# klasmodin/quflow

Measured on AMD Instinct MI355X. Metric: isospectral timesteps/sec at N=1024 (1 GPU) + ensemble steps/sec at 1/2/4/8 GPUs, higher is better.
Workload: dtype f64

## Files before the change

### include/quflow_hip.h

```cpp
#ifndef QUFLOW_HIP_H
#define QUFLOW_HIP_H

#ifdef __cplusplus
extern "C" {
#endif

#define QF_OK 0
#define QF_ERR_INVALID 1
#define QF_ERR_NO_DEVICE 2
#define QF_ERR_HIP 3
#define QF_ERR_STATE 4
#define QF_ERR_CALLBACK 5
#define QF_ERR_UNSUPPORTED 6
#define QF_ERR_NONFINITE 7

#define QF_VERSION 100

typedef struct qf_ctx qf_ctx;

int qf_version(void);
const char *qf_last_error(void);
int qf_device_count(void);

int qf_ctx_create(int N, int device, qf_ctx **out);
// ... 96 lines not shown
#define QF_KERNEL_UPDATE 4
#define QF_KERNEL_SLICE 5
#define QF_KERNEL_COUNT 6

int qf_profile_enable(qf_ctx *ctx, int mask);
int qf_profile_reset(qf_ctx *ctx);
int qf_profile_read(qf_ctx *ctx, int kernel_id, long long *launches, double *total_ms);
int qf_profile_stride(qf_ctx *ctx, int stride);
int qf_profile_seen(qf_ctx *ctx, int kernel_id, long long *seen);
int qf_device_info(int device, char *buf, int n);
int qf_plan_describe(qf_ctx *ctx, char *buf, int n);
int qf_timer_start(qf_ctx *ctx);
int qf_timer_stop(qf_ctx *ctx, double *elapsed_ms);

#define QF_BUF_W 0
#define QF_BUF_DW 1
#define QF_BUF_WHALF 2
#define QF_BUF_PHALF 3
#define QF_BUF_PW 4
int qf_download_buffer(qf_ctx *ctx, int which, void *host);
int qf_debug_guard_check(long long *allocations, long long *damaged, char *first, int n);
int qf_debug_modulus(qf_ctx *ctx, int n, const double *er_host, const double *ei_host, double *out_modulus_host,
                     double *out_sqrt_host);
int qf_zgemm(qf_ctx *ctx, const void *A_host, const void *B_host, void *C_host);
int qf_commutator(qf_ctx *ctx, const void *W_host, const void *P_host, void *C_host, int skewherm);
int qf_zgemm_i8(qf_ctx *ctx, const void *A_host, const void *B_host, void *C_host);
int qf_fixedpoint_products(qf_ctx *ctx, const void *Phalf_host, const void *Whalf_host, const void *W_host,
                           const void *dW_old_host, int variant, void *dW_new_host, void *Whalf_new_host,
                           double *rowsum_host);

int qf_c64_laplacian_table(qf_ctx *ctx, int bc, float *lap_host);
int qf_c64_solve_poisson(qf_ctx *ctx, const void *W_host, void *P_host, int skewh);
int qf_c64_solve_tridiagonal(qf_ctx *ctx, const float *lap_host, const void *W_host, void *P_host, int skewh);
int qf_c64_laplace(qf_ctx *ctx, const void *P_host, void *W_host);
int qf_c64_upload_W(qf_ctx *ctx, const void *W_host);
int qf_c64_download_W(qf_ctx *ctx, void *W_host);
int qf_c64_isomp(qf_ctx *ctx, double dt, int steps, double tol, int minit, int maxit, int compsum, int reinitialize,
                 qf_isomp_stats *stats_out);
int qf_c64_isomp_continue(qf_ctx *ctx, double dt, int steps, double tol, int minit, int maxit, int compsum, int reinitialize,
                          qf_isomp_stats *stats_out);
int qf_c64_diagnostics(qf_ctx *ctx, double *energy_euler, double *enstrophy);
int qf_cgemm(qf_ctx *ctx, const void *A_host, const void *B_host, void *C_host);
int qf_c64_fixedpoint_products(qf_ctx *ctx, const void *Phalf_host, const void *Whalf_host, const void *W_host,
                               const void *dW_old_host, void *dW_new_host, void *Whalf_new_host, double *rowsum_host);
int qf_c64_fixedpoint_products_tri(qf_ctx *ctx, const void *Phalf_host, const void *Whalf_host, const void *W_host,
                                   const void *dW_old_host, void *dW_new_host, void *Whalf_new_host, double *rowsum_host);
// ... 14 lines not shown
```

### quflow_amd/_lib.py

```python
import ctypes
import os

_HERE = os.path.dirname(os.path.abspath(__file__))
LIB_PATH = os.environ.get("QUFLOW_HIP_LIB") or os.path.join(_HERE, "libquflow_hip.so")

QF_OK = 0
QF_ERR_NONFINITE = 7
ERR_NAMES = {1: "QF_ERR_INVALID", 2: "QF_ERR_NO_DEVICE", 3: "QF_ERR_HIP", 4: "QF_ERR_STATE", 5: "QF_ERR_CALLBACK",
             6: "QF_ERR_UNSUPPORTED", 7: "QF_ERR_NONFINITE"}

KERNEL_IDS = {"poisson": 0, "gemm1": 1, "gemm2": 2, "norm": 3, "update": 4, "slice": 5}
ERK_METHODS = {"euler": 0, "heun": 1, "rk4": 2}
BUFFER_IDS = {"W": 0, "dW": 1, "Whalf": 2, "Phalf": 3, "PW": 4}


class QuflowHipError(RuntimeError):
    pass


HAMILTONIAN_CB = ctypes.CFUNCTYPE(ctypes.c_int, ctypes.c_void_p, ctypes.c_void_p, ctypes.c_void_p, ctypes.c_double)
FORCING_CB = ctypes.CFUNCTYPE(ctypes.c_int, ctypes.c_void_p, ctypes.c_void_p, ctypes.c_void_p, ctypes.c_void_p, ctypes.c_double)
STRANG_CB = ctypes.CFUNCTYPE(ctypes.c_int, ctypes.c_void_p, ctypes.c_double, ctypes.c_void_p)
CALLBACK_CB = ctypes.CFUNCTYPE(ctypes.c_int, ctypes.c_void_p, ctypes.c_void_p, ctypes.c_void_p)

# ... 76 lines not shown
                                            ctypes.POINTER(IsompHooks)]),
    "qf_basis_upload": (ctypes.c_int, [_vp, _vp, ctypes.c_longlong]),
    "qf_basis_compute": (ctypes.c_int, [_vp]),
    "qf_basis_download": (ctypes.c_int, [_vp, _vp, ctypes.c_longlong]),
    "qf_basis_stream": (ctypes.c_int, [_vp, ctypes.c_longlong]),
    "qf_basis_slab_plan": (ctypes.c_int, [ctypes.c_int, ctypes.c_int, ctypes.c_longlong, ctypes.POINTER(ctypes.c_int),
                                          ctypes.c_int]),
    "qf_shr2mat": (ctypes.c_int, [_vp, _vp, ctypes.c_longlong, _vp]),
    "qf_mat2shr": (ctypes.c_int, [_vp, _vp, _vp, ctypes.c_longlong]),
    "qf_shc2mat": (ctypes.c_int, [_vp, _vp, _vp]),
    "qf_mat2shc": (ctypes.c_int, [_vp, _vp, _vp]),
    "qf_shr2fun": (ctypes.c_int, [_vp, _vp, ctypes.c_longlong, ctypes.c_int, ctypes.c_int, _vp]),
    "qf_shc2fun": (ctypes.c_int, [_vp, _vp, ctypes.c_longlong, ctypes.c_int, ctypes.c_int, ctypes.c_int, _vp]),
    "qf_fun2shc": (ctypes.c_int, [_vp, _vp, ctypes.c_int, ctypes.c_int, _vp]),
    "qf_fun2shr": (ctypes.c_int, [_vp, _vp, ctypes.c_int, ctypes.c_int, _vp]),
    "qf_diagnostics": (ctypes.c_int, [_vp, _dp, _dp]),
    "qf_norm_inf_W": (ctypes.c_int, [_vp, _dp]),
    "qf_profile_enable": (ctypes.c_int, [_vp, ctypes.c_int]),
    "qf_profile_reset": (ctypes.c_int, [_vp]),
    "qf_profile_read": (ctypes.c_int, [_vp, ctypes.c_int, ctypes.POINTER(ctypes.c_longlong), _dp]),
    "qf_plan_describe": (ctypes.c_int, [_vp, ctypes.c_char_p, ctypes.c_int]),
    "qf_device_info": (ctypes.c_int, [ctypes.c_int, ctypes.c_char_p, ctypes.c_int]),
    "qf_debug_modulus": (ctypes.c_int, [_vp, ctypes.c_int, _dp, _dp, _dp, _dp]),
    "qf_profile_stride": (ctypes.c_int, [_vp, ctypes.c_int]),
    "qf_profile_seen": (ctypes.c_int, [_vp, ctypes.c_int, ctypes.POINTER(ctypes.c_longlong)]),
    "qf_timer_start": (ctypes.c_int, [_vp]),
    "qf_timer_stop": (ctypes.c_int, [_vp, _dp]),
    "qf_download_buffer": (ctypes.c_int, [_vp, ctypes.c_int, _vp]),
    "qf_debug_guard_check": (ctypes.c_int, [ctypes.POINTER(ctypes.c_longlong), ctypes.POINTER(ctypes.c_longlong), ctypes.c_char_p, ctypes.c_int]),
    "qf_zgemm": (ctypes.c_int, [_vp, _vp, _vp, _vp]),
    "qf_commutator": (ctypes.c_int, [_vp, _vp, _vp, _vp, ctypes.c_int]),
    "qf_zgemm_i8": (ctypes.c_int, [_vp, _vp, _vp, _vp]),
    "qf_fixedpoint_products": (ctypes.c_int, [_vp, _vp, _vp, _vp, _vp, ctypes.c_int, _vp, _vp, _vp]),
    "qf_c64_laplacian_table": (ctypes.c_int, [_vp, ctypes.c_int, _vp]),
    "qf_c64_solve_poisson": (ctypes.c_int, [_vp, _vp, _vp, ctypes.c_int]),
    "qf_c64_laplace": (ctypes.c_int, [_vp, _vp, _vp]),
    "qf_c64_solve_tridiagonal": (ctypes.c_int, [_vp, _vp, _vp, _vp, ctypes.c_int]),
    "qf_c64_upload_W": (ctypes.c_int, [_vp, _vp]),
    "qf_c64_download_W": (ctypes.c_int, [_vp, _vp]),
    "qf_c64_isomp": (ctypes.c_int, [_vp, ctypes.c_double, ctypes.c_int, ctypes.c_double, ctypes.c_int,
                                    ctypes.c_int, ctypes.c_int, ctypes.c_int, ctypes.POINTER(IsompStats)]),
    "qf_c64_isomp_continue": (ctypes.c_int, [_vp, ctypes.c_double, ctypes.c_int, ctypes.c_double, ctypes.c_int,
                                             ctypes.c_int, ctypes.c_int, ctypes.c_int, ctypes.POINTER(IsompStats)]),
    "qf_c64_diagnostics": (ctypes.c_int, [_vp, _dp, _dp]),
    "qf_cgemm": (ctypes.c_int, [_vp, _vp, _vp, _vp]),
    "qf_c64_fixedpoint_products": (ctypes.c_int, [_vp, _vp, _vp, _vp, _vp, _vp, _vp, _vp]),
# ... 45 lines not shown
```

### quflow_amd/csrc/api_context.hip

```cpp
#include <cmath>
#include <cstdarg>
#include <cstdio>
#include <cstdlib>
#include <cstring>
#include <limits>
#include <chrono>

#include "qf_api.h"

static thread_local char g_err[512] = "";

void qf_set_error(const char *fmt, ...)
{
    va_list ap;
    va_start(ap, fmt);
    vsnprintf(g_err, sizeof(g_err), fmt, ap);
    va_end(ap);
}

extern "C" {

int qf_version(void) { return QF_VERSION; }

int qf_device_info(int device, char *buf, int n)
// ... 133 lines not shown
    ctx->rowpart_tiles = qf_gemm_tiles_n(N);
    {
        const int slots32 = (N + 31) / 32;
        QF_CREATE_HIP(hipMalloc((void **)&ctx->rowpart, (size_t)(ctx->rowpart_tiles > slots32 ? ctx->rowpart_tiles : slots32) * N * sizeof(double)));
    }
    QF_CREATE_HIP(hipMalloc((void **)&ctx->rowsum, (size_t)N * sizeof(double)));
    QF_CREATE_HIP(hipMalloc((void **)&ctx->scalars, 4096 * sizeof(double)));
    QF_CREATE_HIP(hipHostMalloc((void **)&ctx->host_scalars, 64 * sizeof(double), hipHostMallocDefault));
    QF_CREATE_HIP(hipMalloc((void **)&ctx->state, sizeof(qf_dev_state)));
    QF_CREATE_HIP(hipMemsetAsync(ctx->state, 0, sizeof(qf_dev_state), ctx->stream));
    QF_CREATE_HIP(hipMalloc((void **)&ctx->ticket, 704 * sizeof(unsigned)));
    QF_CREATE_HIP(hipMemsetAsync(ctx->ticket, 0, 704 * sizeof(unsigned), ctx->stream));
    QF_CREATE_HIP(hipHostMalloc((void **)&ctx->host_rec, sizeof(qf_host_record), hipHostMallocCoherent));
    memset(ctx->host_rec, 0, sizeof(qf_host_record));
    {
        hipDeviceProp_t prop;
        QF_CREATE_HIP(hipGetDeviceProperties(&prop, device));
        ctx->num_cus = prop.multiProcessorCount;
        if (N % 64 == 0 && ctx->num_cus > 0) {
            ctx->sk_slots = ctx->num_cus;
            QF_CREATE_HIP(hipMalloc((void **)&ctx->sk_partial, (size_t)ctx->sk_slots * 64 * 64 * sizeof(cplx)));
            QF_CREATE_HIP(hipMalloc((void **)&ctx->sk_flags, (size_t)(ctx->sk_slots + 16) * sizeof(unsigned)));
            QF_CREATE_HIP(hipMemsetAsync(ctx->sk_flags, 0, (size_t)(ctx->sk_slots + 16) * sizeof(unsigned), ctx->stream));
        }
    }
    QF_CREATE_HIP(hipEventCreate(&ctx->timer_start));
    QF_CREATE_HIP(hipEventCreate(&ctx->timer_stop));
#undef QF_CREATE_HIP
    if ((rc = alloc_factors(ctx, &ctx->poisson)) != QF_OK) return fail(rc);
    if ((rc = qf_launch_lap_table(ctx, 1, ctx->lap)) != QF_OK) return fail(rc);
    if ((rc = qf_launch_build_factors(ctx, ctx->lap, ctx->poisson)) != QF_OK) return fail(rc);
    if (hipStreamSynchronize(ctx->stream) != hipSuccess) {
        qf_set_error("qf_ctx_create: table construction failed");
        return fail(QF_ERR_HIP);
    }
    *out = ctx;
    return QF_OK;
}

int qf_ctx_destroy(qf_ctx *ctx)
{
    if (!ctx) return QF_OK;
    (void)hipSetDevice(ctx->device);
    if (ctx->stream) (void)hipStreamSynchronize(ctx->stream);
    void *ptrs[] = {ctx->W, ctx->dW[0], ctx->dW[1], ctx->Whalf, ctx->Phalf, ctx->PW, ctx->kahan_c, ctx->stage,
                    ctx->lap, ctx->lap_user, ctx->poisson.tab, ctx->rowpart, ctx->rowsum,
                    ctx->t32_partial, ctx->t32_arrive, ctx->W2, ctx->Whalf2, ctx->ns_inv, ctx->ns_tmp, ctx->multi_rowpart, ctx->scalars, ctx->sk_partial, ctx->sk_flags, ctx->basis, ctx->sh_stage, ctx->sh_omega, ctx->slab};
    for (void *p : ptrs)
        if (p) (void)hipFree(p);
    void *sht[] = {ctx->sht.omega, ctx->sht.tab, ctx->sht.col, ctx->sht.At, ctx->sht.tw, ctx->sht.f, ctx->sht.H, ctx->sht.Q};
    for (void *p : sht)
        if (p) (void)hipFree(p);
    for (cplx *p : ctx->multi)
        if (p) (void)hipFree(p);
    for (int q = 0; q < 4; ++q) {
        if (ctx->oz_planes[q]) (void)hipFree(ctx->oz_planes[q]);
        if (ctx->oz_scale[q]) (void)hipFree(ctx->oz_scale[q]);
        if (q == 0 && ctx->oz_tbuf) (void)hipFree(ctx->oz_tbuf);
        if (q == 0 && ctx->oz_tflags) (void)hipFree(ctx->oz_tflags);
        if (q == 0 && ctx->oz_diag) (void)hipFree(ctx->oz_diag);
    }
    for (auto &kv : ctx->user_factors) {
        if (kv.second.f.tab) (void)hipFree(kv.second.f.tab);
    }
    for (int q = 0; q < 3; ++q)
        if (ctx->hook_host[q]) (void)hipHostFree(ctx->hook_host[q]);
    qf_c64_free(ctx->c64);
    ctx->c64 = nullptr;
    if (ctx->host_scalars) (void)hipHostFree(ctx->host_scalars);
    if (ctx->host_rec) (void)hipHostFree(ctx->host_rec);
// ... 160 lines not shown
int qf_download_buffer(qf_ctx *ctx, int which, void *host)
{
    QF_TRY(check_ctx(ctx));
    const cplx *src = nullptr;
    switch (which) {
        case QF_BUF_W: src = ctx->W; break;
        case QF_BUF_DW: src = ctx->dW[ctx->dw_cur]; break;
        case QF_BUF_WHALF: src = ctx->Whalf; break;
        case QF_BUF_PHALF: src = ctx->Phalf; break;
        case QF_BUF_PW: src = ctx->PW; break;
        default:
            qf_set_error("qf_download_buffer: unknown buffer %d", which);
            return QF_ERR_INVALID;
    }
    if (!host) {
        qf_set_error("qf_download_buffer: null host pointer");
        return QF_ERR_INVALID;
    }
    QF_HIP(hipMemcpyAsync(host, src, (size_t)ctx->N * ctx->N * sizeof(cplx), hipMemcpyDeviceToHost, ctx->stream));
    QF_HIP(hipStreamSynchronize(ctx->stream));
    return QF_OK;
}

int qf_debug_modulus(qf_ctx *ctx, int n, const double *er_host, const double *ei_host, double *out_modulus_host,
                     double *out_sqrt_host)
{
    QF_TRY(check_ctx(ctx));
    if (n < 1 || (size_t)n > (size_t)ctx->N * ctx->N || !er_host || !ei_host || !out_modulus_host || !out_sqrt_host) {
        qf_set_error("qf_debug_modulus: bad arguments (n=%d)", n);
        return QF_ERR_INVALID;
    }
    double *d = reinterpret_cast<double *>(ctx->stage), *o = reinterpret_cast<double *>(ctx->PW);
    QF_HIP(hipMemcpyAsync(d, er_host, (size_t)n * sizeof(double), hipMemcpyHostToDevice, ctx->stream));
    QF_HIP(hipMemcpyAsync(d + n, ei_host, (size_t)n * sizeof(double), hipMemcpyHostToDevice, ctx->stream));
    QF_TRY(qf_launch_debug_modulus(ctx, n, d, d + n, o, o + n));
    QF_HIP(hipMemcpyAsync(out_modulus_host, o, (size_t)n * sizeof(double), hipMemcpyDeviceToHost, ctx->stream));
    QF_HIP(hipMemcpyAsync(out_sqrt_host, o + n, (size_t)n * sizeof(double), hipMemcpyDeviceToHost, ctx->stream));
    QF_HIP(hipStreamSynchronize(ctx->stream));
    return QF_OK;
}


}
```

### quflow_amd/csrc/qf_internal.h

```cpp
#pragma once

#include <hip/hip_runtime.h>

#include <atomic>
#include <cstdarg>
#include <cstdio>
#include <map>
#include <mutex>
#include <string>
#include <vector>

#include "../../include/quflow_hip.h"

typedef double2 cplx;

hipError_t qf_guard_malloc(void **p, size_t bytes);
hipError_t qf_guard_free(void *p);
#define hipMalloc(p, n) qf_guard_malloc((void **)(p), (n))
#define hipFree(p) qf_guard_free((void *)(p))

void qf_set_error(const char *fmt, ...);
struct qf_ctx;
inline void qf_plan_note(qf_ctx *ctx, unsigned long long key, const char *fmt, ...) __attribute__((format(printf, 3, 4)));

// ... 255 lines not shown
    int rowpart_tiles = 0;
    double *rowsum = nullptr;
    double *scalars = nullptr;
    double *host_scalars = nullptr;
    qf_dev_state *state = nullptr;
    qf_host_record *host_rec = nullptr;
    bool diag_at_exit = false, diag_valid = false;
    unsigned *ticket = nullptr;
    int pred_iters = 3;
    bool gemm_tri_allowed = true;
    bool gemm_tri = false;
    int gemm_tri_min_n = 960;
    bool gemm_tri32 = false;
    int tri32_split = 2, tri32_split_diag = 1;
    cplx *t32_partial = nullptr;
    unsigned *t32_arrive = nullptr;
    bool defer_allowed = true;
    bool defer = false;
    int num_cus = 0;
    cplx *sk_partial = nullptr;
    unsigned *sk_flags = nullptr;
    int sk_slots = 0;
    unsigned sk_epoch = 0;
    int sk_epi_units = 0;
    int sk_epi_units_fused = 2;
    int sk_min_units = 8;
    int debug_drop = 0;
    bool needs_reset = false;

    qf_c64 *c64 = nullptr;

    int profile_mask = 0;
    std::vector<qf_event_pair> events_busy;
    std::vector<qf_event_pair> events_free;
    int profile_stride = 1;
    struct plan_slot {
        unsigned long long key = 0;
        char text[384] = {0};
    } plan[QF_KERNEL_COUNT];
    int plan_role = -1;
    long long prof_seen[QF_KERNEL_COUNT] = {0};
    long long prof_launches[QF_KERNEL_COUNT] = {0};
    double prof_ms[QF_KERNEL_COUNT] = {0};
    hipEvent_t timer_start = nullptr, timer_stop = nullptr;
};

// ... 37 lines not shown
    cplx *Whalf = nullptr;
    double *rowpart = nullptr;
    int fused = 0;
    cplx *Wpair[2] = {nullptr, nullptr};
    cplx *Whalf_step = nullptr;
    unsigned *ticket = nullptr;
    int n_tiles = 0;
    qf_dev_state *state_rw = nullptr;
    qf_host_record *rec = nullptr;
    int debug_drop = 0;
};
struct qf_streamk {
    cplx *partial = nullptr;
    unsigned *flags = nullptr;
    unsigned epoch = 0;
    int *fault = nullptr;
    unsigned *ticket = nullptr;
    int n_tiles = 0;
    qf_dev_state *state_rw = nullptr;
    qf_host_record *rec = nullptr;
    unsigned spin_limit = 1u << 22;
    int debug_drop = 0;
    int slots = 0;
};
struct qf_tri32 {
    cplx *partial = nullptr;
    unsigned *arrive = nullptr;
    int split = 1;
    int split_diag = 1;
    unsigned *ticket = nullptr;
    int n_tiles = 0;
    qf_dev_state *state_rw = nullptr;
    qf_host_record *rec = nullptr;
    int debug_drop = 0;
    int deferred = 0;
};
int qf_gemm_tiles_n(int N);
int qf_launch_zgemm_tri32(qf_ctx *ctx, const cplx *A, const cplx *B, const qf_epilogue *ep, qf_guard guard = qf_guard());
int qf_launch_zgemm_tri(qf_ctx *ctx, const cplx *A, const cplx *B, const qf_epilogue *ep, qf_guard guard = qf_guard());
int qf_launch_zgemm(qf_ctx *ctx, const cplx *A, const cplx *B, cplx *C, const qf_epilogue *ep,
                    qf_guard guard = qf_guard());

int qf_launch_basis(qf_ctx *ctx, double *basis_dev);
__host__ __device__ inline long long qf_slab_prefix(int N, int Nmax, int m)
{
    const long long a = m, n = N, k = Nmax;
    return a * n * k - (n + k) * (a * (a - 1) / 2) + (a - 1) * a * (2 * a - 1) / 6;
// ... 64 lines not shown
```

### quflow_amd/csrc/qf_step_end.h

```cpp
#pragma once

#include "qf_internal.h"

template <int ROWS = 4>
__device__ inline void qf_fused_step_end(int N, int slots, const double *rowpart, unsigned *ticket, qf_dev_state *state,
                                  qf_host_record *rec, int g_iter, int tid, double *scratch)
{
    double *part = scratch;
    int *nanflag = reinterpret_cast<int *>(scratch + 4);
    const bool check = (g_iter + 1 >= state->minit);
    double mx = 0.0;
    int nan = 0;
    if (check) {
        typedef unsigned v2u __attribute__((ext_vector_type(2)));
        const __amdgpu_buffer_rsrc_t rs_rp = __builtin_amdgcn_make_buffer_rsrc(
            const_cast<double *>(rowpart), 0, (int)((size_t)slots * N * sizeof(double)), 0x00020000);
        const unsigned slot_bytes = (unsigned)((size_t)N * sizeof(double));
        for (int ib = tid; ib < N; ib += ROWS * 256) {
            double sum[ROWS];
#pragma unroll
            for (int r = 0; r < ROWS; ++r) sum[r] = 0.0;
            for (int t0 = 0; t0 < slots; t0 += 16) {
                v2u v[ROWS][16];
#pragma unroll
                for (int r = 0; r < ROWS; ++r) {
// ... 7 lines not shown
#pragma unroll
                for (int r = 0; r < ROWS; ++r)
#pragma unroll
                    for (int t = 0; t < 16; ++t)
                        if (t0 + t < slots) sum[r] += *reinterpret_cast<const double *>(&v[r][t]);
            }
#pragma unroll
            for (int r = 0; r < ROWS; ++r)
                if (ib + 256 * r < N) {
                    if (sum[r] != sum[r]) nan = 1; else mx = fmax(mx, sum[r]);
                }
        }
#pragma unroll
        for (int off = 32; off > 0; off >>= 1) {
            mx = fmax(mx, __shfl_xor(mx, off, 64));
            nan |= __shfl_xor(nan, off, 64);
        }
        if ((tid & 63) == 0) {
            part[tid >> 6] = mx;
            nanflag[tid >> 6] = nan;
        }
    }
    __syncthreads();
    if (tid == 0) {
        __hip_atomic_store(ticket, 0u, __ATOMIC_RELAXED, __HIP_MEMORY_SCOPE_AGENT);
        const int iters = g_iter + 1;
        state->total_iterations += 1;
        state->dw_parity ^= 1;
        bool done = false, aborted = false;
        if (check) {
            double r = fmax(fmax(part[0], part[1]), fmax(part[2], part[3]));
            if (nanflag[0] | nanflag[1] | nanflag[2] | nanflag[3]) r = __builtin_nan("");
            const double resnorm_old = state->resnorm;
            state->resnorm = r;
            if (!QF_FINITE(r)) aborted = true;
            if (r <= state->tol || r >= resnorm_old) done = true;
        }
        if (aborted) {
            rec->nonfinite = 1;
            rec->last_step_iters = iters;
            rec->resnorm = state->resnorm;
            state->step_index = QF_STEP_ABORTED;
            state->iters_this_step = 0;
            state->wh_sel = 0;
        } else if (done || iters >= state->maxit) {
            if (!done) state->number_of_maxit += 1;
            rec->last_step_iters = iters;
            rec->resnorm = state->resnorm;
            state->step_index += 1;
            state->iters_this_step = 0;
            state->resnorm = __builtin_inf();
            state->w_parity ^= 1;
            state->wh_sel = 1;
        } else {
            state->iters_this_step = iters;
            state->wh_sel = 0;
        }
        rec->total_iterations = state->total_iterations;
        rec->number_of_maxit = state->number_of_maxit;
        rec->step_index = state->step_index;
        rec->w_parity = state->w_parity;
        rec->wh_sel = state->wh_sel;
        rec->dw_parity = state->dw_parity;
        const unsigned long long prog = ((unsigned long long)(unsigned)state->step_index << 32) |
                                        (unsigned long long)(unsigned)state->iters_this_step;
        __hip_atomic_store(&rec->progress, prog, __ATOMIC_RELEASE, __HIP_MEMORY_SCOPE_SYSTEM);
    }
}



struct qf_new_state {
    int step_index, iters_this_step, wh_sel, w_parity, dw_parity;
    int closed, last_step_iters, hit_maxit;
    int nonfinite;
    double resnorm;
    double last_resnorm;
};

__device__ inline qf_new_state qf_decide_compute(int N, int slots, const double *__restrict__ rowpart,
                                                 const qf_dev_state *st, double *scratch)
{
    const int tid = threadIdx.x, nth = blockDim.x, nw = nth >> 6;
    double *part = scratch;
    int *nanflag = reinterpret_cast<int *>(scratch + 20);
    const int iters = st->pending_iter + 1;
    const int minit = st->minit, maxit = st->maxit;
    const double tol = st->tol, resnorm_old = st->resnorm;
    const int step_index = st->step_index, w_parity = st->w_parity, dw_parity = st->dw_parity;
    const bool check = iters >= minit;
    double r = 0.0;
    {
        double mx = 0.0;
// ... 102 lines not shown
```

### quflow_amd/csrc/zgemm.hip

```cpp
#include "qf_internal.h"
#include "qf_step_end.h"

#include <cstring>

typedef double v4d __attribute__((ext_vector_type(4)));

#ifdef QF_STAMP
__device__ unsigned long long *qf_stamp_buf = nullptr;
#define QF_STAMP_SLOTS 80
#ifdef QF_STAMP_LIGHT
#define QF_STAMP_AT(slot_)
#define QF_STAMP_PH(kt_, ph_)
__device__ unsigned long long *qf_phase_buf = nullptr;
#else
#define QF_STAMP_AT(slot_)                                                              \
    if (qf_stamp_buf && lane == 0 && (slot_) < QF_STAMP_SLOTS)                          \
        qf_stamp_buf[((size_t)blockIdx.x * (T / 64) + wave) * QF_STAMP_SLOTS + (slot_)] = __builtin_amdgcn_s_memtime();
__device__ unsigned long long *qf_phase_buf = nullptr;
#define QF_STAMP_PH(kt_, ph_)                                                           \
    if (qf_phase_buf && tid == 0 && (kt_) >= 20 && (kt_) < 28)                          \
        qf_phase_buf[((size_t)blockIdx.x * 8 + ((kt_) - 20)) * 5 + (ph_)] = __builtin_amdgcn_s_memtime();
#endif
__device__ unsigned long long *qf_tri_buf = nullptr;
#define QF_TRI_STAMP(seg_, k_)                                                          \
    if (qf_tri_buf && tid == 0 && (seg_) < 4)                                           \
        qf_tri_buf[((size_t)blockIdx.x * 4 + (seg_)) * 8 + (k_)] = __builtin_amdgcn_s_memtime();
#define QF_TRI_NOTE(seg_, k_, v_)                                                       \
    if (qf_tri_buf && tid == 0 && (seg_) < 4) qf_tri_buf[((size_t)blockIdx.x * 4 + (seg_)) * 8 + (k_)] = (unsigned long long)(v_);
#else
#define QF_STAMP_AT(slot_)
#define QF_STAMP_PH(kt_, ph_)
#define QF_TRI_STAMP(seg_, k_)
#define QF_TRI_NOTE(seg_, k_, v_)
#endif
#ifndef QF_ABL_NOSTORE
#define QF_ABL_NOSTORE 0
#endif
#ifndef QF_ABL_NOSUMS
#define QF_ABL_NOSUMS 0
#endif
#ifndef QF_ABL_NOADD
#define QF_ABL_NOADD 0
#endif
#define QF_SUM3M(c_) (QF_ABL_NOADD ? (c_).x : (c_).x + (c_).y)
#ifndef QF_ABL_NOGLOAD
#define QF_ABL_NOGLOAD 0
#endif
#ifndef QF_ABL_NOBARRIER
#define QF_ABL_NOBARRIER 0
#endif
#ifndef QF_SK_AUX_ST
// ... 803 lines not shown
                            }
                        }
                    }
                    asm volatile("s_barrier" ::: "memory");
                    const unsigned soff = (unsigned)((size_t)slot2 * (BM * BN) * sizeof(cplx));
                    cplx v[MT * NT * 4];
#pragma unroll
                    for (int q = 0; q < MT * NT * 4; ++q) {
                        const v4u raw = __builtin_amdgcn_raw_buffer_load_b128(rsrcP, p_voff + (unsigned)(q * T * sizeof(cplx)), soff, QF_SK_AUX_LD);
                        v[q] = *reinterpret_cast<const cplx *>(&raw);
                    }
#pragma unroll
                    for (int mi = 0; mi < MT; ++mi)
#pragma unroll
                        for (int ni = 0; ni < NT; ++ni)
#pragma unroll
                            for (int reg = 0; reg < 4; ++reg) {
                                tre[mi][ni][reg] += v[(mi * NT + ni) * 4 + reg].x;
                                tim[mi][ni][reg] += v[(mi * NT + ni) * 4 + reg].y;
                            }
                }
            }
            QF_TRI_STAMP(seg, 2)
            cplx *Th = reinterpret_cast<cplx *>(smem_raw);
            cplx *Ts = reinterpret_cast<cplx *>(smem_raw + TT_BYTES);
            double *rs = reinterpret_cast<double *>(smem_raw + 2 * TT_BYTES);
            double *cs = rs + WN * BM;
            unsigned *open_flag = reinterpret_cast<unsigned *>(cs + WM * BN);
            const bool offdiag = (tm != tn);
            asm volatile("s_waitcnt lgkmcnt(0)\n\ts_barrier" ::: "memory");

            double csum[NT] = {0.0, 0.0};
            if (tid == 0) *open_flag = 0u;
#pragma unroll
            for (int mi = 0; mi < MT; ++mi) {
#pragma unroll
                for (int reg = 0; reg < 4; ++reg) {
                    const int li = wm * WTM + mi * 16 + q4 + 4 * reg;
                    double rsum = 0.0;
#pragma unroll
                    for (int ni = 0; ni < NT; ++ni) {
                        const int lj = wn * WTN + ni * 16 + r16;
                        const size_t e = (size_t)(i0 + li) * N + (j0 + lj);
                        const double dr = tre[mi][ni][reg] + e_c[mi][ni][reg].x;
                        const double di = tim[mi][ni][reg] + e_c[mi][ni][reg].y;
                        tre[mi][ni][reg] = dr;
// ... 4 lines not shown
                        ep.Whalf[e] = wh;
                        Th[li * TS + lj] = wh;
                        if (!ep.fused) Ts[li * TS + lj] = make_double2(dr, di);
                        const cplx o = e_old[mi][ni][reg];
                        const double er = o.x - dr, ei = o.y - di;
                        const double a = qf_modulus(er, ei);
                        rsum += a;
                        csum[ni] += a;
                    }
                    rsum = qf_row16_sum(rsum);
                    if (r16 == 0) rs[wn * BM + li] = rsum;
                }
            }
            if (offdiag) {
#pragma unroll
                for (int ni = 0; ni < NT; ++ni) {
                    double s2 = csum[ni];
                    s2 += __shfl_xor(s2, 16, 64);
                    s2 += __shfl_xor(s2, 32, 64);
                    if (q4 == 0) cs[wm * BN + wn * WTN + ni * 16 + r16] = s2;
                }
            }
            asm volatile("s_waitcnt lgkmcnt(0)\n\ts_barrier" ::: "memory");
            if (tid < BM) {
                double s2 = 0.0;
#pragma unroll
                for (int cc = 0; cc < WN; ++cc) s2 += rs[cc * BM + tid];
                __hip_atomic_store(ep.rowpart + (size_t)tn * N + i0 + tid, s2, __ATOMIC_RELAXED, __HIP_MEMORY_SCOPE_AGENT);
                if (open_if_large && s2 > tol_now) *open_flag = 1u;
            } else if (offdiag && tid < BM + BN) {
                const int lj = tid - BM;
                double s2 = 0.0;
#pragma unroll
                for (int cc = 0; cc < WM; ++cc) s2 += cs[cc * BN + lj];
                __hip_atomic_store(ep.rowpart + (size_t)tm * N + j0 + lj, s2, __ATOMIC_RELAXED, __HIP_MEMORY_SCOPE_AGENT);
                if (open_if_large && s2 > tol_now) *open_flag = 1u;
            }
            unsigned ticket_old = 0u;
            if (ep.fused) {
                asm volatile("s_waitcnt vmcnt(0) lgkmcnt(0)\n\ts_barrier" ::: "memory");
                if (tid == 0 && !((sk.debug_drop & 2) && t == 0))
                    ticket_old = __hip_atomic_fetch_add(sk.ticket, 1u, __ATOMIC_RELAXED, __HIP_MEMORY_SCOPE_AGENT);
            } else {
                asm volatile("s_waitcnt lgkmcnt(0)\n\ts_barrier" ::: "memory");
            }
            QF_TRI_STAMP(seg, 7)
            const bool speculate = ep.fused && !(open_for_sure || (open_if_large && *open_flag != 0u));

            if (speculate) {
#pragma unroll
                for (int mi = 0; mi < MT; ++mi)
#pragma unroll
                    for (int reg = 0; reg < 4; ++reg) {
                        const int li = wm * WTM + mi * 16 + q4 + 4 * reg;
#pragma unroll
                        for (int ni = 0; ni < NT; ++ni) {
                            const int lj = wn * WTN + ni * 16 + r16;
                            const size_t e = (size_t)(i0 + li) * N + (j0 + lj);
                            const cplx w = e_w[mi][ni][reg];
                            const cplx wc = make_double2(w.x + 2.0 * e_c[mi][ni][reg].x, w.y + 2.0 * e_c[mi][ni][reg].y);
                            const cplx whs = make_double2(wc.x + tre[mi][ni][reg], wc.y + tim[mi][ni][reg]);
                            ep_Wnext[e] = wc;
                            ep.Whalf_step[e] = whs;
                            Ts[li * TS + lj] = whs;
                        }
                    }
            }
            asm volatile("s_waitcnt lgkmcnt(0)\n\ts_barrier" ::: "memory");
            if (offdiag) {
#pragma unroll
                for (int r = 0; r < 16; ++r) {
                    const int jl = wave * 16 + r;
                    const cplx wv = Th[lane_v * TS + jl];
                    const size_t e2 = (size_t)(j0 + jl) * N + (i0 + lane_v);
                    ep.Whalf[e2] = make_double2(-wv.x, wv.y);
                    if (speculate || !ep.fused) {
                        const cplx ws = Ts[lane_v * TS + jl];
                        if (ep.fused) ep.Whalf_step[e2] = make_double2(-ws.x, ws.y);
                        else ep_dW_new[e2] = make_double2(-ws.x, ws.y);
                    }
                }
            }
            if (have_next) QF_TRI_START_LOADS(n_k0, n_KT, n_tm, n_tn)
            if (ep.fused) {
                unsigned *last_flag = reinterpret_cast<unsigned *>(rs);
                if (tid == 0) *last_flag = (ticket_old == (unsigned)(sk.n_tiles - 1)) ? 1u : 0u;
                asm volatile("s_waitcnt lgkmcnt(0)\n\ts_barrier" ::: "memory");
                if (*last_flag != 0u) run_finale = true;
            }
        }
        QF_TRI_STAMP(seg, 3)
        ++seg;
        have = have_next;
        t = n_t;
        k0 = n_k0;
        KT = n_KT;
        tm = n_tm;
        tn = n_tn;
        asm volatile("s_waitcnt lgkmcnt(0)\n\ts_barrier" ::: "memory");
    }
    if (run_finale)
        qf_fused_step_end(N, nt, ep.rowpart, sk.ticket, sk.state_rw, sk.rec, guard.iter, tid, reinterpret_cast<double *>(smem_raw));
#undef QF_TRI_NEXT
#undef QF_TRI_KOF
#undef QF_TRI_HAS_PIECE
#undef QF_TRI_START_LOADS
}

template <bool EXACT>
__global__ __launch_bounds__(256) void k_zgemm_tri32(int N, int nt, const cplx *__restrict__ A, const cplx *__restrict__ B,
                                                      qf_epilogue ep, qf_guard guard, qf_tri32 sx)
{
    if (!qf_guard_iter(guard)) return;
    constexpr int BM = 32, BN = 32, WM = 2, WN = 2;
    constexpr bool EPI = true, FAST = false;
    using SM = tile_smem<BM, BN, false>;
    constexpr int T = WM * WN * 64;
    constexpr int WTM = BM / WM, WTN = BN / WN;
    constexpr int MT = WTM / 16, NT = WTN / 16;
    static_assert(MT == 1 && NT == 1, "one MFMA tile per wave");
    constexpr int A_STRIDE = SM::A_STRIDE, B_STRIDE = SM::B_STRIDE;
    constexpr int A_PER = (BM * BK) / T, B_PER = (BN * BK) / T;
    constexpr int A_ROWS_PER = T / BK, B_ROWS_PER = T / BN;
    constexpr int A3_STRIDE = SM::A3_STRIDE, B3_STRIDE = SM::B3_STRIDE;
    constexpr int TS = BN + 1;
// ... 372 lines not shown
    if (!ep || N % 64 != 0 || !ctx->sk_partial || ctx->num_cus < 1) {
        qf_set_error("qf_launch_zgemm_tri: not available for this context (N=%d)", N);
        return QF_ERR_STATE;
    }
    static qf_smem_attr attr;
    QF_TRY(qf_smem_attr_set(attr, (const void *)k_zgemm_tri, ctx->device, TRI_SMEM_BYTES));
    const int nt = N / 64;
    int E = ep->fused ? ctx->sk_epi_units_fused : ctx->sk_epi_units;
    if (E < -8) E = -8;
    const long long units = (long long)nt * (nt + 1) / 2 * (N / BK + E);
    if (units > 0x7fffffffLL) {
        qf_set_error("qf_launch_zgemm_tri: N=%d is too large for the stream-K partition", N);
        return QF_ERR_INVALID;
    }
    long long grid_ll = units / (ctx->sk_min_units > 0 ? ctx->sk_min_units : 1);
    if (grid_ll > ctx->num_cus) grid_ll = ctx->num_cus;
    if (grid_ll < 1) grid_ll = 1;
    const int grid = (int)grid_ll;
    qf_streamk sk;
    const int slots = ctx->sk_slots > 0 ? ctx->sk_slots : ctx->num_cus;
    sk.slots = slots;
    sk.partial = ctx->sk_partial;
    sk.flags = ctx->sk_flags;
    sk.epoch = ++ctx->sk_epoch;
    sk.fault = &ctx->host_rec->fault;
    sk.ticket = ctx->sk_flags + slots;
    sk.n_tiles = nt * (nt + 1) / 2;
    sk.state_rw = ctx->state;
    sk.rec = ctx->host_rec;
    if (ctx->debug_drop == 1 || (ctx->debug_drop == 2 && ep->fused)) {
        sk.debug_drop = ctx->debug_drop;
        sk.spin_limit = 1u << 14;
        ctx->debug_drop = 0;
    }
    qf_plan_note(ctx, 0x2000000ull | (unsigned long long)(grid << 8 | (E & 0x3f) << 1 | (ep->fused ? 1 : 0)),
                 "{\"kernel\": \"k_zgemm_tri\", \"arithmetic\": \"fp64 3M, v_mfma_f64_16x16x4_f64\", \"tile\": [64, 64], \"tiles\": %d, "
                 "\"tile_share\": %.6f, \"workgroups\": %d, \"threads\": 256, \"partition\": \"stream-K over (tile, K-tile) units, "
                 "contiguous ranges, epilogue weight E = %d K-tiles\", \"step_end\": \"%s\"}",
                 sk.n_tiles, (double)sk.n_tiles / ((double)nt * nt), grid, E, ep->fused ? "fused (last finisher decides)" : "two-kernel");
    hipLaunchKernelGGL(k_zgemm_tri, dim3(grid), dim3(256), TRI_SMEM_BYTES, ctx->stream, N, nt, (int)units, E, A, B, *ep, guard, sk);
    QF_HIP(hipGetLastError());
    return QF_OK;
}

int qf_launch_zgemm_tri32(qf_ctx *ctx, const cplx *A, const cplx *B, const qf_epilogue *ep, qf_guard guard)
{
    const int N = ctx->N;
// ... 44 lines not shown
```

Before: 2696.

## Replace ticket fence with epoch-tagged row-sum granules in fused step end

In the fused stream-K triangular ZGEMM epilogue, row and column partial sums are now written as epoch-tagged 32-bit halves into a per-context granule buffer. The ticket increment moves ahead of the epilogue and no longer waits behind a vmcnt(0) barrier. The last finisher's step-end reduction spins until every granule carries the current epoch before reducing. This removes the store-drain barrier on every tile, at the cost of doubled row-sum traffic, a validation spin loop in the finale, and a new device buffer. It also adds debug hooks and widens the timing-stamp layout.

```diff
diff --git a/include/quflow_hip.h b/include/quflow_hip.h
--- a/include/quflow_hip.h
+++ b/include/quflow_hip.h
@@ -142,6 +142,8 @@
 int qf_debug_guard_check(long long *allocations, long long *damaged, char *first, int n);
 int qf_debug_modulus(qf_ctx *ctx, int n, const double *er_host, const double *ei_host, double *out_modulus_host,
                      double *out_sqrt_host);
+unsigned qf_debug_sk_next_epoch(unsigned prev);
+long long qf_debug_sk_rowgran(qf_ctx *ctx, void *host, long long nbytes, unsigned *epoch);
 int qf_zgemm(qf_ctx *ctx, const void *A_host, const void *B_host, void *C_host);
 int qf_commutator(qf_ctx *ctx, const void *W_host, const void *P_host, void *C_host, int skewherm);
 int qf_zgemm_i8(qf_ctx *ctx, const void *A_host, const void *B_host, void *C_host);
diff --git a/quflow_amd/_lib.py b/quflow_amd/_lib.py
--- a/quflow_amd/_lib.py
+++ b/quflow_amd/_lib.py
@@ -122,6 +122,8 @@
     "qf_plan_describe": (ctypes.c_int, [_vp, ctypes.c_char_p, ctypes.c_int]),
     "qf_device_info": (ctypes.c_int, [ctypes.c_int, ctypes.c_char_p, ctypes.c_int]),
     "qf_debug_modulus": (ctypes.c_int, [_vp, ctypes.c_int, _dp, _dp, _dp, _dp]),
+    "qf_debug_sk_next_epoch": (ctypes.c_uint, [ctypes.c_uint]),
+    "qf_debug_sk_rowgran": (ctypes.c_longlong, [_vp, _vp, ctypes.c_longlong, ctypes.POINTER(ctypes.c_uint)]),
     "qf_profile_stride": (ctypes.c_int, [_vp, ctypes.c_int]),
     "qf_profile_seen": (ctypes.c_int, [_vp, ctypes.c_int, ctypes.POINTER(ctypes.c_longlong)]),
     "qf_timer_start": (ctypes.c_int, [_vp]),
diff --git a/quflow_amd/csrc/api_context.hip b/quflow_amd/csrc/api_context.hip
--- a/quflow_amd/csrc/api_context.hip
+++ b/quflow_amd/csrc/api_context.hip
@@ -179,6 +179,9 @@
             QF_CREATE_HIP(hipMalloc((void **)&ctx->sk_partial, (size_t)ctx->sk_slots * 64 * 64 * sizeof(cplx)));
             QF_CREATE_HIP(hipMalloc((void **)&ctx->sk_flags, (size_t)(ctx->sk_slots + 16) * sizeof(unsigned)));
             QF_CREATE_HIP(hipMemsetAsync(ctx->sk_flags, 0, (size_t)(ctx->sk_slots + 16) * sizeof(unsigned), ctx->stream));
+            const size_t gran_bytes = qf_sk_rowgran_bytes(N);
+            QF_CREATE_HIP(hipMalloc((void **)&ctx->sk_rowgran, gran_bytes));
+            QF_CREATE_HIP(hipMemsetAsync(ctx->sk_rowgran, 0, gran_bytes, ctx->stream));
         }
     }
     QF_CREATE_HIP(hipEventCreate(&ctx->timer_start));
@@ -202,7 +205,7 @@
     if (ctx->stream) (void)hipStreamSynchronize(ctx->stream);
     void *ptrs[] = {ctx->W, ctx->dW[0], ctx->dW[1], ctx->Whalf, ctx->Phalf, ctx->PW, ctx->kahan_c, ctx->stage,
                     ctx->lap, ctx->lap_user, ctx->poisson.tab, ctx->rowpart, ctx->rowsum,
-                    ctx->t32_partial, ctx->t32_arrive, ctx->W2, ctx->Whalf2, ctx->ns_inv, ctx->ns_tmp, ctx->multi_rowpart, ctx->scalars, ctx->sk_partial, ctx->sk_flags, ctx->basis, ctx->sh_stage, ctx->sh_omega, ctx->slab};
+                    ctx->t32_partial, ctx->t32_arrive, ctx->W2, ctx->Whalf2, ctx->ns_inv, ctx->ns_tmp, ctx->multi_rowpart, ctx->scalars, ctx->sk_partial, ctx->sk_flags, ctx->sk_rowgran, ctx->basis, ctx->sh_stage, ctx->sh_omega, ctx->slab};
     for (void *p : ptrs)
         if (p) (void)hipFree(p);
     void *sht[] = {ctx->sht.omega, ctx->sht.tab, ctx->sht.col, ctx->sht.At, ctx->sht.tw, ctx->sht.f, ctx->sht.H, ctx->sht.Q};
@@ -409,6 +412,24 @@
     return QF_OK;
 }
 
+unsigned qf_debug_sk_next_epoch(unsigned prev) { return qf_sk_next_epoch(prev); }
+
+long long qf_debug_sk_rowgran(qf_ctx *ctx, void *host, long long nbytes, unsigned *epoch)
+{
+    if (const int rc = check_ctx(ctx)) return -rc;
+    if (epoch) *epoch = ctx->sk_epoch;
+    if (!ctx->sk_rowgran) return 0;
+    const long long have = (long long)qf_sk_rowgran_bytes(ctx->N);
+    if (host && nbytes > 0) {
+        if (hipMemcpyAsync(host, ctx->sk_rowgran, (size_t)(nbytes < have ? nbytes : have), hipMemcpyDeviceToHost, ctx->stream) != hipSuccess ||
+            hipStreamSynchronize(ctx->stream) != hipSuccess) {
+            qf_set_error("qf_debug_sk_rowgran: the copy failed");
+            return -QF_ERR_HIP;
+        }
+    }
+    return have;
+}
+
 int qf_debug_modulus(qf_ctx *ctx, int n, const double *er_host, const double *ei_host, double *out_modulus_host,
                      double *out_sqrt_host)
 {
diff --git a/quflow_amd/csrc/qf_internal.h b/quflow_amd/csrc/qf_internal.h
--- a/quflow_amd/csrc/qf_internal.h
+++ b/quflow_amd/csrc/qf_internal.h
@@ -301,6 +301,7 @@
     unsigned *sk_flags = nullptr;
     int sk_slots = 0;
     unsigned sk_epoch = 0;
+    unsigned long long *sk_rowgran = nullptr;
     int sk_epi_units = 0;
     int sk_epi_units_fused = 2;
     int sk_min_units = 8;
@@ -384,7 +385,14 @@
     unsigned spin_limit = 1u << 22;
     int debug_drop = 0;
     int slots = 0;
-};
+    unsigned long long *rowgran = nullptr;
+};
+inline unsigned qf_sk_next_epoch(unsigned prev)
+{
+    const unsigned e = prev + 1u;
+    return e != 0u ? e : 1u;
+}
+inline size_t qf_sk_rowgran_bytes(int N) { return (size_t)(N / 64) * N * 2 * sizeof(unsigned long long); }
 struct qf_tri32 {
     cplx *partial = nullptr;
     unsigned *arrive = nullptr;
diff --git a/quflow_amd/csrc/qf_step_end.h b/quflow_amd/csrc/qf_step_end.h
--- a/quflow_amd/csrc/qf_step_end.h
+++ b/quflow_amd/csrc/qf_step_end.h
@@ -1,6 +1,53 @@
 #pragma once
 
 #include "qf_internal.h"
+
+__device__ inline void qf_step_end_decide(bool check, const double *part, const int *nanflag, unsigned *ticket,
+                                          qf_dev_state *state, qf_host_record *rec, int g_iter)
+{
+    __hip_atomic_store(ticket, 0u, __ATOMIC_RELAXED, __HIP_MEMORY_SCOPE_AGENT);
+    const int iters = g_iter + 1;
+    state->total_iterations += 1;
+    state->dw_parity ^= 1;
+    bool done = false, aborted = false;
+    if (check) {
+        double r = fmax(fmax(part[0], part[1]), fmax(part[2], part[3]));
+        if (nanflag[0] | nanflag[1] | nanflag[2] | nanflag[3]) r = __builtin_nan("");
+        const double resnorm_old = state->resnorm;
+        state->resnorm = r;
+        if (!QF_FINITE(r)) aborted = true;
+        if (r <= state->tol || r >= resnorm_old) done = true;
+    }
+    if (aborted) {
+        rec->nonfinite = 1;
+        rec->last_step_iters = iters;
+        rec->resnorm = state->resnorm;
+        state->step_index = QF_STEP_ABORTED;
+        state->iters_this_step = 0;
+        state->wh_sel = 0;
+    } else if (done || iters >= state->maxit) {
+        if (!done) state->number_of_maxit += 1;
+        rec->last_step_iters = iters;
+        rec->resnorm = state->resnorm;
+        state->step_index += 1;
+        state->iters_this_step = 0;
+        state->resnorm = __builtin_inf();
+        state->w_parity ^= 1;
+        state->wh_sel = 1;
+    } else {
+        state->iters_this_step = iters;
+        state->wh_sel = 0;
+    }
+    rec->total_iterations = state->total_iterations;
+    rec->number_of_maxit = state->number_of_maxit;
+    rec->step_index = state->step_index;
+    rec->w_parity = state->w_parity;
+    rec->wh_sel = state->wh_sel;
+    rec->dw_parity = state->dw_parity;
+    const unsigned long long prog = ((unsigned long long)(unsigned)state->step_index << 32) |
+                                    (unsigned long long)(unsigned)state->iters_this_step;
+    __hip_atomic_store(&rec->progress, prog, __ATOMIC_RELEASE, __HIP_MEMORY_SCOPE_SYSTEM);
+}
 
 template <int ROWS = 4>
 __device__ inline void qf_fused_step_end(int N, int slots, const double *rowpart, unsigned *ticket, qf_dev_state *state,
@@ -54,53 +101,87 @@
         }
     }
     __syncthreads();
-    if (tid == 0) {
-        __hip_atomic_store(ticket, 0u, __ATOMIC_RELAXED, __HIP_MEMORY_SCOPE_AGENT);
-        const int iters = g_iter + 1;
-        state->total_iterations += 1;
-        state->dw_parity ^= 1;
-        bool done = false, aborted = false;
-        if (check) {
-            double r = fmax(fmax(part[0], part[1]), fmax(part[2], part[3]));
-            if (nanflag[0] | nanflag[1] | nanflag[2] | nanflag[3]) r = __builtin_nan("");
-            const double resnorm_old = state->resnorm;
-            state->resnorm = r;
-            if (!QF_FINITE(r)) aborted = true;
-            if (r <= state->tol || r >= resnorm_old) done = true;
-        }
-        if (aborted) {
-            rec->nonfinite = 1;
-            rec->last_step_iters = iters;
-            rec->resnorm = state->resnorm;
-            state->step_index = QF_STEP_ABORTED;
-            state->iters_this_step = 0;
-            state->wh_sel = 0;
-        } else if (done || iters >= state->maxit) {
-            if (!done) state->number_of_maxit += 1;
-            rec->last_step_iters = iters;
-            rec->resnorm = state->resnorm;
-            state->step_index += 1;
-            state->iters_this_step = 0;
-            state->resnorm = __builtin_inf();
-            state->w_parity ^= 1;
-            state->wh_sel = 1;
-        } else {
-            state->iters_this_step = iters;
-            state->wh_sel = 0;
-        }
-        rec->total_iterations = state->total_iterations;
-        rec->number_of_maxit = state->number_of_maxit;
-        rec->step_index = state->step_index;
-        rec->w_parity = state->w_parity;
-        rec->wh_sel = state->wh_sel;
-        rec->dw_parity = state->dw_parity;
-        const unsigned long long prog = ((unsigned long long)(unsigned)state->step_index << 32) |
-                                        (unsigned long long)(unsigned)state->iters_this_step;
-        __hip_atomic_store(&rec->progress, prog, __ATOMIC_RELEASE, __HIP_MEMORY_SCOPE_SYSTEM);
-    }
-}
-
-
+    if (tid == 0) qf_step_end_decide(check, part, nanflag, ticket, state, rec, g_iter);
+}
+
+template <int ROWS = 4>
+__device__ inline unsigned qf_fused_step_end_inband(int N, int slots, const unsigned long long *gran, unsigned epoch,
+                                                    unsigned spin_limit, int *fault, unsigned *ticket, qf_dev_state *state,
+                                                    qf_host_record *rec, int g_iter, int tid, double *scratch)
+{
+    double *part = scratch;
+    int *nanflag = reinterpret_cast<int *>(scratch + 4);
+    int *stale = reinterpret_cast<int *>(scratch + 6);
+    const bool check = (g_iter + 1 >= state->minit);
+    double mx = 0.0;
+    int nan = 0;
+    unsigned sweeps = 0;
+    if (check) {
+        typedef unsigned v4u __attribute__((ext_vector_type(4)));
+        const __amdgpu_buffer_rsrc_t rs_g = __builtin_amdgcn_make_buffer_rsrc(
+            const_cast<unsigned long long *>(gran), 0, (int)((size_t)slots * N * 16), 0x00020000);
+        const unsigned slot_bytes = (unsigned)((size_t)N * 16);
+        for (;;) {
+            ++sweeps;
+            if (tid == 0) *stale = 0;
+            __syncthreads();
+            mx = 0.0;
+            nan = 0;
+            bool ok = true;
+            for (int ib = tid; ib < N; ib += ROWS * 256) {
+                double sum[ROWS];
+#pragma unroll
+                for (int r = 0; r < ROWS; ++r) sum[r] = 0.0;
+                for (int t0 = 0; t0 < slots; t0 += 16) {
+                    v4u v[ROWS][16];
+#pragma unroll
+                    for (int r = 0; r < ROWS; ++r) {
+                        const unsigned vo = (unsigned)(((ib + 256 * r < N) ? ib + 256 * r : ib) * 16);
+#pragma unroll
+                        for (int t = 0; t < 16; ++t) {
+                            const unsigned so = (t0 + t < slots) ? (unsigned)(t0 + t) * slot_bytes : 0u;
+                            v[r][t] = __builtin_amdgcn_raw_buffer_load_b128(rs_g, vo, so, 16);
+                        }
+                    }
+#pragma unroll
+                    for (int r = 0; r < ROWS; ++r)
+#pragma unroll
+                        for (int t = 0; t < 16; ++t) {
+                            ok &= (v[r][t].y == epoch) & (v[r][t].w == epoch);
+                            const unsigned long long bits = ((unsigned long long)v[r][t].z << 32) | v[r][t].x;
+                            if (t0 + t < slots) sum[r] += __builtin_bit_cast(double, bits);
+                        }
+                }
+#pragma unroll
+                for (int r = 0; r < ROWS; ++r)
+                    if (ib + 256 * r < N) {
+                        if (sum[r] != sum[r]) nan = 1; else mx = fmax(mx, sum[r]);
+                    }
+            }
+            if (!ok) *stale = 1;
+            __syncthreads();
+            if (*stale == 0) break;
+            if (sweeps > spin_limit) {
+                if (tid == 0) *fault = 1;
+                break;
+            }
+            __builtin_amdgcn_s_sleep(8);
+            __syncthreads();
+        }
+#pragma unroll
+        for (int off = 32; off > 0; off >>= 1) {
+            mx = fmax(mx, __shfl_xor(mx, off, 64));
+            nan |= __shfl_xor(nan, off, 64);
+        }
+        if ((tid & 63) == 0) {
+            part[tid >> 6] = mx;
+            nanflag[tid >> 6] = nan;
+        }
+    }
+    __syncthreads();
+    if (tid == 0) qf_step_end_decide(check, part, nanflag, ticket, state, rec, g_iter);
+    return sweeps;
+}
 
 struct qf_new_state {
     int step_index, iters_this_step, wh_sel, w_parity, dw_parity;
diff --git a/quflow_amd/csrc/zgemm.hip b/quflow_amd/csrc/zgemm.hip
--- a/quflow_amd/csrc/zgemm.hip
+++ b/quflow_amd/csrc/zgemm.hip
@@ -24,9 +24,9 @@
 __device__ unsigned long long *qf_tri_buf = nullptr;
 #define QF_TRI_STAMP(seg_, k_)                                                          \
     if (qf_tri_buf && tid == 0 && (seg_) < 4)                                           \
-        qf_tri_buf[((size_t)blockIdx.x * 4 + (seg_)) * 8 + (k_)] = __builtin_amdgcn_s_memtime();
+        qf_tri_buf[((size_t)blockIdx.x * 4 + (seg_)) * 16 + (k_)] = __builtin_amdgcn_s_memtime();
 #define QF_TRI_NOTE(seg_, k_, v_)                                                       \
-    if (qf_tri_buf && tid == 0 && (seg_) < 4) qf_tri_buf[((size_t)blockIdx.x * 4 + (seg_)) * 8 + (k_)] = (unsigned long long)(v_);
+    if (qf_tri_buf && tid == 0 && (seg_) < 4) qf_tri_buf[((size_t)blockIdx.x * 4 + (seg_)) * 16 + (k_)] = (unsigned long long)(v_);
 #else
 #define QF_STAMP_AT(slot_)
 #define QF_STAMP_PH(kt_, ph_)
@@ -876,6 +876,10 @@
                 }
             }
             QF_TRI_STAMP(seg, 2)
+            unsigned ticket_old = 0u;
+            if (ep.fused && tid == 0 && !((sk.debug_drop & 2) && t == 0))
+                ticket_old = __builtin_amdgcn_atomic_inc32(sk.ticket, 0xffffffffu, __ATOMIC_RELAXED, "agent");
+            QF_TRI_STAMP(seg, 9)
             cplx *Th = reinterpret_cast<cplx *>(smem_raw);
             cplx *Ts = reinterpret_cast<cplx *>(smem_raw + TT_BYTES);
             double *rs = reinterpret_cast<double *>(smem_raw + 2 * TT_BYTES);
@@ -926,28 +930,30 @@
                 }
             }
             asm volatile("s_waitcnt lgkmcnt(0)\n\ts_barrier" ::: "memory");
-            if (tid < BM) {
+            if (tid < BM + BN && (tid < BM || offdiag)) {
+                const bool row = tid < BM;
+                const int l = row ? tid : tid - BM;
                 double s2 = 0.0;
-#pragma unroll
-                for (int cc = 0; cc < WN; ++cc) s2 += rs[cc * BM + tid];
-                __hip_atomic_store(ep.rowpart + (size_t)tn * N + i0 + tid, s2, __ATOMIC_RELAXED, __HIP_MEMORY_SCOPE_AGENT);
-                if (open_if_large && s2 > tol_now) *open_flag = 1u;
-            } else if (offdiag && tid < BM + BN) {
-                const int lj = tid - BM;
-                double s2 = 0.0;
-#pragma unroll
-                for (int cc = 0; cc < WM; ++cc) s2 += cs[cc * BN + lj];
-                __hip_atomic_store(ep.rowpart + (size_t)tm * N + j0 + lj, s2, __ATOMIC_RELAXED, __HIP_MEMORY_SCOPE_AGENT);
+                if (row) {
+#pragma unroll
+                    for (int cc = 0; cc < WN; ++cc) s2 += rs[cc * BM + l];
+                } else {
+#pragma unroll
+                    for (int cc = 0; cc < WM; ++cc) s2 += cs[cc * BN + l];
+                }
+                const size_t at = row ? (size_t)tn * N + i0 + l : (size_t)tm * N + j0 + l;
+                if (ep.fused) {
+                    const unsigned long long bits = __builtin_bit_cast(unsigned long long, s2);
+                    const unsigned long long tag = (unsigned long long)sk.epoch << 32;
+                    __hip_atomic_store(sk.rowgran + 2 * at, tag | (bits & 0xffffffffull), __ATOMIC_RELAXED, __HIP_MEMORY_SCOPE_AGENT);
+                    __hip_atomic_store(sk.rowgran + 2 * at + 1, tag | (bits >> 32), __ATOMIC_RELAXED, __HIP_MEMORY_SCOPE_AGENT);
+                } else {
+                    __hip_atomic_store(ep.rowpart + at, s2, __ATOMIC_RELAXED, __HIP_MEMORY_SCOPE_AGENT);
+                }
                 if (open_if_large && s2 > tol_now) *open_flag = 1u;
             }
-            unsigned ticket_old = 0u;
-            if (ep.fused) {
-                asm volatile("s_waitcnt vmcnt(0) lgkmcnt(0)\n\ts_barrier" ::: "memory");
-                if (tid == 0 && !((sk.debug_drop & 2) && t == 0))
-                    ticket_old = __hip_atomic_fetch_add(sk.ticket, 1u, __ATOMIC_RELAXED, __HIP_MEMORY_SCOPE_AGENT);
-            } else {
-                asm volatile("s_waitcnt lgkmcnt(0)\n\ts_barrier" ::: "memory");
-            }
+            QF_TRI_STAMP(seg, 8)
+            asm volatile("s_waitcnt lgkmcnt(0)\n\ts_barrier" ::: "memory");
             QF_TRI_STAMP(seg, 7)
             const bool speculate = ep.fused && !(open_for_sure || (open_if_large && *open_flag != 0u));
 
@@ -989,6 +995,7 @@
             if (ep.fused) {
                 unsigned *last_flag = reinterpret_cast<unsigned *>(rs);
                 if (tid == 0) *last_flag = (ticket_old == (unsigned)(sk.n_tiles - 1)) ? 1u : 0u;
+                QF_TRI_STAMP(seg, 10)
                 asm volatile("s_waitcnt lgkmcnt(0)\n\ts_barrier" ::: "memory");
                 if (*last_flag != 0u) run_finale = true;
             }
@@ -1003,8 +1010,14 @@
         tn = n_tn;
         asm volatile("s_waitcnt lgkmcnt(0)\n\ts_barrier" ::: "memory");
     }
-    if (run_finale)
-        qf_fused_step_end(N, nt, ep.rowpart, sk.ticket, sk.state_rw, sk.rec, guard.iter, tid, reinterpret_cast<double *>(smem_raw));
+    if (run_finale) {
+        QF_TRI_STAMP(0, 12)
+        const unsigned sweeps = qf_fused_step_end_inband<2>(N, nt, sk.rowgran, sk.epoch, sk.spin_limit, sk.fault, sk.ticket, sk.state_rw,
+                                                         sk.rec, guard.iter, tid, reinterpret_cast<double *>(smem_raw));
+        (void)sweeps;
+        QF_TRI_STAMP(0, 13)
+        QF_TRI_NOTE(0, 14, sweeps)
+    }
 #undef QF_TRI_NEXT
 #undef QF_TRI_KOF
 #undef QF_TRI_HAS_PIECE
@@ -1423,7 +1436,12 @@
     sk.slots = slots;
     sk.partial = ctx->sk_partial;
     sk.flags = ctx->sk_flags;
-    sk.epoch = ++ctx->sk_epoch;
+    sk.epoch = ctx->sk_epoch = qf_sk_next_epoch(ctx->sk_epoch);
+    sk.rowgran = ctx->sk_rowgran;
+    if (ep->fused && !sk.rowgran) {
+        qf_set_error("qf_launch_zgemm_tri: the fused step end needs the context's row-sum granules");
+        return QF_ERR_STATE;
+    }
     sk.fault = &ctx->host_rec->fault;
     sk.ticket = ctx->sk_flags + slots;
     sk.n_tiles = nt * (nt + 1) / 2;
```

After: 2686. About the same (-0.4%).
